# vmonardo/pnp-svrg

Measured on AMD Instinct MI355X. Metric: PnP-SVRG inner-iters/sec, 256x256 CSMRI+DnCNN, higher is better.
Workload: dtype f32; 1 GPU; pnp_svrg (true SVRG direction, T2=10, mb=1000) on 256x256 CSMRI, 20% Bernoulli mask, DnCNN-17 prox (reference DnCNN_noise15 weights); batch_per_gpu=120, problems_total=120, parallelism=replicas x1 (no data-path collective)

## Files before the change

### pnp_svrg_amd/csrc/dncnn.hip

```cpp
#include "direct.h"
#include "wino44.h"
#include "wino44b.h"
#include "reduce.h"
#include <vector>
#include <algorithm>
#include <cstdlib>
#include <type_traits>

namespace pnp {

constexpr int C = 64;

template <typename T>
__global__ __launch_bounds__(256) void k_first(const T* __restrict__ z, const T* __restrict__ mm,
                                               const float* __restrict__ w, const float* __restrict__ bfirst,
                                               float* __restrict__ out, int H, int W, double srange, double sshift,
                                               int clamp01, float slope) {
    __shared__ float ws[C * 9];
    __shared__ float bs[C];
    for (int i = threadIdx.x; i < C * 9; i += 256) ws[i] = w[i];
    if (threadIdx.x < C) bs[threadIdx.x] = bfirst[threadIdx.x];
    __syncthreads();
    const int b = blockIdx.y;
    const int p = blockIdx.x * 256 + threadIdx.x;
// ... 140 lines not shown
                                                      float blast) {
    __shared__ double red[4];
    const int tid = threadIdx.x, b = blockIdx.z;
    const int iy = tid >> 6, ix = tid & 3, bx = blockIdx.x * 16 + ((tid >> 2) & 15), by = blockIdx.y;
    const int y = 4 * by + iy, x = 4 * bx + ix;
    const int NBX = W / 4, NBY = H / 4;
    const float* pb = part + (size_t)b * NBY * NBX * 36;
    auto at = [&](int qy, int qx, int py, int px) { return pb[((size_t)qy * NBX + qx) * 36 + py * 6 + px]; };
    const int vy = iy == 0 ? -1 : iy == 3 ? 1 : 0, vx = ix == 0 ? -1 : ix == 3 ? 1 : 0;
    const bool hv = vy != 0 && by + vy >= 0 && by + vy < NBY, hh = vx != 0 && bx + vx >= 0 && bx + vx < NBX;
    const int py = iy + 1, px = ix + 1, pyn = py - 4 * vy, pxn = px - 4 * vx;
    float r = at(by, bx, py, px);
    if (hv) r += at(by + vy, bx, pyn, px);
    if (hh) r += at(by, bx + vx, py, pxn);
    if (hv && hh) r += at(by + vy, bx + vx, pyn, pxn);
    r += blast;
    const size_t p = (size_t)b * H * W + (size_t)y * W + x;
    if (r_out != nullptr) r_out[p] = r;
    double err = 0.0;
    if (zout != nullptr) {
        const T lo = mm ? mm[2 * b] : (T)0, hi = mm ? mm[2 * b + 1] : (T)1;
        T v = (zin[p] - lo) / (hi - lo);
        v = v * (T)srange + (T)sshift;
        v = v - (T)r;
        v = (v - (T)sshift) / (T)srange;
        v = v * (hi - lo) + lo;
        zout[p] = v;
        if (xrec != nullptr) {
            const double d = (double)xrec[p] - (double)v;
            err = d * d;
        }
    }
    if (sse_part != nullptr) {
        err = wave_sum(err);
        if ((tid & 63) == 0) red[tid >> 6] = err;
        __syncthreads();
        if (tid == 0)
            sse_part[((size_t)b * gridDim.y + blockIdx.y) * gridDim.x + blockIdx.x] = red[0] + red[1] + red[2] + red[3];
    }
}

__global__ void k_sum_parts(const double* __restrict__ part, int nparts, double* __restrict__ out) {
    double s = 0;
    for (int i = threadIdx.x; i < nparts; i += 64) s += part[(size_t)blockIdx.x * nparts + i];
    s = wave_sum(s);
    if (threadIdx.x == 0) out[blockIdx.x] = s;
}

}
using namespace pnp;

static const ConvMode kModes[] = {
    {0, direct_supports, direct_layer_bytes, direct_pack, direct_layer, direct_debug_clock, false},
    {1, direct_supports, wino23_layer_bytes, wino23_pack, wino23_layer, wino23_debug_clock, false},
    {5, wino44_supports, wino44_layer_bytes, wino44_pack, wino44_layer, wino44_debug_clock, true},
    {6, wino44b_supports, wino44b_layer_bytes, wino44b_pack, wino44b_layer, wino44b_debug_clock, false},
};
constexpr int NMODES = sizeof(kModes) / sizeof(kModes[0]);

static const ConvMode* find_mode(int mode) {
    for (const ConvMode& m : kModes)
        if (m.mode == mode) return &m;
    return nullptr;
}

static int resolve_conv_mode(int requested, int H, int W, bool strict, const ConvMode** out) {
    const ConvMode* m = find_mode(requested);
    PNP_CHECK_ARG(m || !strict,
                  "mode must be 0 (direct), 1 (Winograd F(2,3) along x), 5 (Winograd F(4x4,3x3)) or 6 (the same on 3 x bf16 splits)");
    if (!m) m = find_mode(5);
    PNP_CHECK_ARG(m->supports(H, W) || !strict, "Winograd F(4x4,3x3) needs H % 8 == 0 and W % 64 == 0");
    *out = m->supports(H, W) ? m : find_mode(1);
    return PNP_OK;
}

struct pnp_dncnn_plan {
    int n_mid, H, W, batch, num_cu;
    float *w_first, *w_last, *bias;
    void* wconv[NMODES];
    const ConvMode* conv;
    float* b_first;
    float b_last, slope;
    bool edge_fusion;
    float* part;
    float *act0, *act1, *zeros;
    double* mm;
    double* sse_part;
    bool profile;
    std::vector<hipEvent_t> ev;
    size_t ev_used;
    double prof_ms;
    long prof_launches;
};

static void plan_free(pnp_dncnn_plan* p) {
    for (void* q : p->wconv) (void)hipFree(q);
    for (void* q : {(void*)p->bias, (void*)p->w_first, (void*)p->w_last, (void*)p->act0, (void*)p->act1, (void*)p->zeros,
                    (void*)p->mm, (void*)p->sse_part, (void*)p->b_first, (void*)p->part})
        (void)hipFree(q);
    for (hipEvent_t e : p->ev) (void)hipEventDestroy(e);
    delete p;
}

static ConvLayerArgs conv_args(const pnp_dncnn_plan* p, int l, const float* in, float* out, hipStream_t s) {
    return {in, out, p->wconv[p->conv - kModes], l, p->bias + (size_t)l * C, p->zeros, p->H, p->W, p->batch, p->num_cu, p->slope, s};
}

extern "C" int pnp_dncnn_plan_create(pnp_dncnn_plan** out, int n_mid, const float* w_first, const float* w_mid,
                                     const float* b_mid, const float* w_last, int H, int W, int batch) {
    PNP_CHECK_ARG(out && w_first && w_mid && b_mid && w_last, "null argument");
    PNP_CHECK_ARG(n_mid >= 1 && batch >= 1, "n_mid and batch must be >= 1");
    PNP_CHECK_ARG(H % 8 == 0 && W % 32 == 0 && (H * W) % 256 == 0, "H must be a multiple of 8, W of 32");
    auto* p = new pnp_dncnn_plan{};
    p->n_mid = n_mid; p->H = H; p->W = W; p->batch = batch;
    hipDeviceProp_t prop;
    int dev = 0;
    PNP_CHECK_HIP(hipGetDevice(&dev));
    PNP_CHECK_HIP(hipGetDeviceProperties(&prop, dev));
    p->num_cu = prop.multiProcessorCount;
    const char* ev = getenv("PNP_DNCNN_WINOGRAD");
    (void)resolve_conv_mode(ev ? atoi(ev) : 5, H, W, false, &p->conv);
    const char* ef = getenv("PNP_DNCNN_EDGE_FUSION");
    p->edge_fusion = !(ef && atoi(ef) == 0);
    const size_t act_bytes = (size_t)batch * C * H * W * sizeof(float);
    hipError_t e = hipSuccess;
    auto alloc = [&](auto** dst, size_t bytes, const void* src = nullptr) {
        if (e == hipSuccess) e = hipMalloc(dst, bytes);
        if (e == hipSuccess && src) e = hipMemcpy(*dst, src, bytes, hipMemcpyHostToDevice);
    };
    for (int i = 0; i < NMODES; ++i) {
        if (!kModes[i].supports(H, W)) continue;
        std::vector<char> w(kModes[i].layer_bytes() * n_mid);
        kModes[i].pack(w_mid, n_mid, w.data());
        alloc(&p->wconv[i], w.size(), w.data());
    }
    alloc(&p->bias, (size_t)n_mid * C * sizeof(float), b_mid);
    alloc(&p->w_first, C * 9 * sizeof(float), w_first);
    alloc(&p->w_last, C * 9 * sizeof(float), w_last);
    alloc(&p->b_first, C * sizeof(float));
    if (e == hipSuccess) e = hipMemset(p->b_first, 0, C * sizeof(float));
    alloc(&p->act0, act_bytes);
    alloc(&p->act1, act_bytes);
    alloc(&p->zeros, 256);
    if (e == hipSuccess) e = hipMemset(p->zeros, 0, 256);
    alloc(&p->mm, (size_t)batch * 2 * sizeof(double));
    alloc(&p->sse_part, (size_t)batch * (H * W / 256) * sizeof(double));
    if (wino44_supports(H, W)) alloc(&p->part, wino44_part_floats(H, W, batch) * sizeof(float));
    if (e != hipSuccess) {
        set_error(std::string("pnp_dncnn_plan_create: ") + hipGetErrorString(e));
        plan_free(p);
        return PNP_ERR_HIP;
    }
    *out = p;
    return PNP_OK;
}

extern "C" int pnp_dncnn_plan_destroy(pnp_dncnn_plan* p) {
    if (p) plan_free(p);
    return PNP_OK;
}

namespace {
template <typename T>
int run_dncnn(pnp_dncnn_plan* p, const T* z_in, bool normalise, double sigma_net, T* z_out, float* r_out,
              const T* xrec, double* sse_out, hipStream_t s, bool mmo = false) {
    const int H = p->H, W = p->W, B = p->batch, HW = H * W;
    T* mm = normalise ? (T*)p->mm : nullptr;
    double srange = 1.0, sshift = 0.0;
    if (normalise) {
        k_minmax<T><<<B, 256, 0, s>>>(z_in, HW, mm);
        PNP_CHECK_LAUNCH();
        srange = 1.0 + sigma_net / 255.0 / 2.0;
        sshift = (1.0 - srange) / 2.0;
    }
    dim3 pg(HW / 256, B);
    k_first<T><<<pg, 256, 0, s>>>(z_in, mm, p->w_first, p->b_first, p->act0, H, W, srange, sshift, mmo ? 1 : 0, p->slope);
    PNP_CHECK_LAUNCH();
    float *src = p->act0, *dst = p->act1;
    const bool fuse_last = p->edge_fusion && p->conv->fuses_last && p->slope == 0.f && !mmo && std::is_same<T, float>::value &&
                           p->part != nullptr;
    const bool prof = p->profile && p->ev_used + 2 <= p->ev.size();
    if (prof) PNP_CHECK_HIP(hipEventRecord(p->ev[p->ev_used], s));
    for (int l = 0; l < p->n_mid; ++l) {
        ConvLayerArgs a = conv_args(p, l, src, dst, s);
        if (fuse_last && l == p->n_mid - 1) { a.wlast = p->w_last; a.part = p->part; }
        const int rc = p->conv->layer(a);
        if (rc != PNP_OK) return rc;
        std::swap(src, dst);
    }
    if (prof) { PNP_CHECK_HIP(hipEventRecord(p->ev[p->ev_used + 1], s)); p->ev_used += 2; }
    if (fuse_last) {
        const dim3 fg(W / 64, H / 4, B);
        k_last_patches<T><<<fg, 256, 0, s>>>(p->part, z_in, mm, z_out, r_out, xrec, sse_out ? p->sse_part : nullptr, H, W, srange,
                                             sshift, p->b_last);
        PNP_CHECK_LAUNCH();
        if (sse_out) {
            k_sum_parts<<<B, 64, 0, s>>>(p->sse_part, (int)(fg.x * fg.y), sse_out);
            PNP_CHECK_LAUNCH();
        }
        return PNP_OK;
    }
    dim3 lg((W + LT_C - 1) / LT_C, (H + LT_R - 1) / LT_R, B);
    k_last<T><<<lg, 256, 0, s>>>(src, p->w_last, z_in, mm, z_out, r_out, xrec, sse_out ? p->sse_part : nullptr, H, W,
                                 srange, sshift, mmo ? 1 : 0, p->b_last);
    PNP_CHECK_LAUNCH();
    if (sse_out) {
// ... 120 lines not shown
```

### pnp_svrg_amd/csrc/dncnn_conv.h

```cpp
#pragma once
#include "common.h"
#include <vector>

namespace pnp {

struct ConvLayerArgs {
    const float* in;
    float* out;
    const void* w;
    int layer;
    const float *bias, *zeros;
    int H, W, batch, num_cu;
    float slope;
    hipStream_t s;
    int force_rows = 0;
    const float* w44_override = nullptr;
    const float* wlast = nullptr;
    float* part = nullptr;
};

struct ConvMode {
    int mode;
    bool (*supports)(int H, int W);
    size_t (*layer_bytes)();
    void (*pack)(const float* w_mid, int n_mid, void* out);
    int (*layer)(const ConvLayerArgs& a);
    int (*debug_clock)(const ConvLayerArgs& a, int reps, std::vector<double>& cycles, std::vector<double>& ticks);
    bool fuses_last;
};

inline int check_plain_conv(const ConvLayerArgs& a) {
    PNP_CHECK_ARG(a.w44_override == nullptr, "w44_override needs the F(4x4,3x3) kernel (mode 5)");
    PNP_CHECK_ARG(a.part == nullptr, "the fused last layer needs the F(4x4,3x3) kernel (mode 5) and ReLU");
    return PNP_OK;
}

template <typename F>
int read_stamps(hipStream_t s, int nwg, int per_wg, F&& launch, std::vector<unsigned long long>& h, std::vector<double>& cycles,
                std::vector<double>& ticks) {
    unsigned long long* d = nullptr;
    PNP_CHECK_HIP(hipMalloc(&d, (size_t)nwg * per_wg * sizeof(*d)));
    h.resize((size_t)nwg * per_wg);
    const int rc = launch(d);
    hipError_t e = rc != PNP_OK ? hipSuccess : hipMemcpyAsync(h.data(), d, h.size() * sizeof(*d), hipMemcpyDeviceToHost, s);
    if (rc == PNP_OK && e == hipSuccess) e = hipStreamSynchronize(s);
    (void)hipFree(d);
    if (rc != PNP_OK) return rc;
    PNP_CHECK_HIP(e);
    for (int i = 0; i < nwg; ++i) { cycles.push_back((double)h[(size_t)per_wg * i]); ticks.push_back((double)h[(size_t)per_wg * i + 1]); }
    return PNP_OK;
}

}
```

### pnp_svrg_amd/csrc/dncnn_wino44.hip

```cpp
#include "common.h"
#include "wino44.h"
#include "wino44_common.h"
#include "tilewalk.h"
#include <vector>
#include <utility>
#include <cstdlib>

namespace pnp {
namespace w44 {

using namespace w44c;

template <int NG_> struct Geo : HaloGeo<NG_> {
    static constexpr int NG = NG_;
    static constexpr int VPL = 128 * NG;
    static constexpr int VBUF = 36 * VPL;
    static constexpr int LDS_FLOATS = 2 * HaloGeo<NG_>::DBUF + 2 * VBUF;
    static constexpr int NQ_AGPR = NG == 2 ? 64 : 36;
    static constexpr bool in_agpr(int g, int xi) { return g * 36 + xi < NQ_AGPR; }
};
constexpr int URING = 18;

#define PNP_MFMA_PRE ""
#define PNP_MFMA_POST ""
template <bool AG> __device__ __forceinline__ void mfma(f32x4& acc, float w, float v) {
    if (AG) asm volatile(PNP_MFMA_PRE "v_mfma_f32_16x16x4_f32 %0, %1, %2, %0" PNP_MFMA_POST : "+a"(acc) : "v"(w), "v"(v));
    else asm volatile(PNP_MFMA_PRE "v_mfma_f32_16x16x4_f32 %0, %1, %2, %0" PNP_MFMA_POST : "+v"(acc) : "v"(w), "v"(v));
}
template <bool AG> __device__ __forceinline__ void mfma_first(f32x4& acc, float w, float v) {
    if (AG) asm volatile("v_mfma_f32_16x16x4_f32 %0, %1, %2, 0" PNP_MFMA_POST : "=&a"(acc) : "v"(w), "v"(v));
    else asm volatile("v_mfma_f32_16x16x4_f32 %0, %1, %2, 0" PNP_MFMA_POST : "=&v"(acc) : "v"(w), "v"(v));
}

template <int NG_> struct Ctx : WeightCursor {
    static constexpr int NG = NG_;
    using G = Geo<NG_>;
    f32x4 acc[NG_][36];
    f32x4 ur[URING];
    Patch P;
    f32x2 b[2][NG_];
    const lds_f* dsrc[2];
    lds_f* vdst[2];
    const lds_f* vsrc0[2];
};
#define PNP_SLOT() __builtin_amdgcn_sched_barrier(0)

constexpr int col_pair(int sl) { return (sl - 6) / 2; }
constexpr bool is_col_slice(int sl) { return sl == 6 || sl == 8 || sl == 10; }
template <int SL, typename CT> __device__ __forceinline__ void slice_valu(CT& c) {
    Patch& P = c.P;
    if constexpr (SL < 6) {
        asm volatile("" :: "v"(P.a.x), "v"(P.e.y));
        const f32x2 p12 = {P.m.x, P.m.y}, p34 = {P.m.z, P.m.w};
        const f32x2 A = p34 - 4.f * p12;
        const f32x2 Bv = p34 - p12;
        P.t[SL][1] = pk_sum_diff(A);
        P.t[SL][2] = pk_hi_pm_2lo(Bv);
        float v0, v5;
        asm("v_fma_f32 %0, 4.0, %1, %2" : "=v"(v0) : "v"(P.a.y), "v"(__builtin_fmaf(-5.f, P.m.y, P.m.w)));
        asm("v_fma_f32 %0, 4.0, %1, %2" : "=v"(v5) : "v"(P.m.x), "v"(__builtin_fmaf(-5.f, P.m.z, P.e.x)));
        P.t[SL][0] = f32x2{v0, v5};
    } else if constexpr (is_col_slice(SL)) {
        constexpr int cp = col_pair(SL);
        bt6_pk(P.t[0][cp], P.t[1][cp], P.t[2][cp], P.t[3][cp], P.t[4][cp], P.t[5][cp], P.v);
    }
}
template <int DPAR, int SL, int Y, typename CT> __device__ __forceinline__ void v_write(CT& c) {
    constexpr int VPL = CT::G::VPL;
    constexpr int cp = col_pair(SL), xa = cp == 0 ? 0 : cp == 1 ? 1 : 3, xb = cp == 0 ? 5 : cp == 1 ? 2 : 4;
    c.vdst[DPAR][(Y * 6 + xa) * VPL] = c.P.v[Y].x;
    c.vdst[DPAR][(Y * 6 + xb) * VPL] = c.P.v[Y].y;
}
template <int DPAR, int SL, int N, typename CT> __device__ __forceinline__ void slice_lds(CT& c) {
    if constexpr (SL < 5) {
        if constexpr (N < 2) patch_load<DPAR, SL + 1, N>(c);
    } else if constexpr (is_col_slice(SL)) {
        v_write<DPAR, SL, 2 * N>(c);
        v_write<DPAR, SL, 2 * N + 1>(c);
    }
}
template <int VPAR, int XI, typename CT> __device__ __forceinline__ void b_load(CT& c) {
    if constexpr (CT::NG == 1) c.b[XI & 1][0] = *(const lds_f2*)(c.vsrc0[VPAR] + XI * CT::G::VPL);
    else {
        const f32x4 q = *(const lds_f4*)(c.vsrc0[VPAR] + XI * CT::G::VPL);
        c.b[XI & 1][0] = f32x2{q.x, q.y};
        c.b[XI & 1][CT::NG - 1] = f32x2{q.z, q.w};
    }
}
template <int K, int XI, int GR, typename CT> __device__ __forceinline__ void mfma_j0(CT& c, float u, f32x2 (&b)[CT::NG]) {
// ... 50 lines not shown
    else if constexpr (P == 7 || P == 9 || P == 11) slice_valu<P - 1>(c);
}
template <int K, int P, int VAR, typename CT, typename DMA> __device__ __forceinline__ void step2(CT& c, DMA&& dma) {
    static_assert(CT::NG == 2 && CT::G::PPW == 6, "one DMA piece in each of the steps 0..5");
    constexpr int X0 = 2 * P, X1 = 2 * P + 1, SQ = K * 18 + P;
    constexpr int VPAR = K & 1, DPAR = (K + 1) & 1;
    const f32x4 u = c.ur[SQ % URING];
    f32x2 b0[2] = {c.b[0][0], c.b[0][1]}, b1[2];
    mfma_j0<K, X0, 0>(c, u.x, b0);                   PNP_SLOT();
    if constexpr (VAR != 13 && VAR != 15) b_load<VPAR, X1>(c);
    PNP_SLOT();
    mfma_j0<K, X0, 1>(c, u.x, b0);                   PNP_SLOT();
    slot2<DPAR, P, 0, VAR>(c, dma);
    PNP_SLOT();
    mfma_j1<X0, 0>(c, u.y, b0);                      PNP_SLOT();
    if constexpr (VAR != 10 && VAR != 15) valu2<P>(c);
    if constexpr (P == 0 && K > 0 && VAR != 12 && VAR != 15 && SQ - 1 + URING < NCH * 18) c.ur[(SQ - 1) % URING] = c.uload_next();
    PNP_SLOT();
    mfma_j1<X0, 1>(c, u.y, b0);                      PNP_SLOT();
    slot2<DPAR, P, 1, VAR>(c, dma);
    PNP_SLOT();
    b1[0] = c.b[1][0]; b1[1] = c.b[1][1];
    mfma_j0<K, X1, 0>(c, u.z, b1);                   PNP_SLOT();
    if constexpr (X1 + 1 < 36 && VAR != 13 && VAR != 15) b_load<VPAR, X1 + 1>(c);
    PNP_SLOT();
    mfma_j0<K, X1, 1>(c, u.z, b1);                   PNP_SLOT();
    slot2<DPAR, P, 2, VAR>(c, dma);
    PNP_SLOT();
    mfma_j1<X1, 0>(c, u.w, b1);                      PNP_SLOT();
    slot2<DPAR, P, 3, VAR>(c, dma);
    PNP_SLOT();
    mfma_j1<X1, 1>(c, u.w, b1);                      PNP_SLOT();
    if constexpr (P < 17 && VAR != 12 && VAR != 15 && SQ + URING < NCH * 18) c.ur[SQ % URING] = c.uload_next();
    PNP_SLOT();
}
template <int K, int VAR, typename CT, typename DMA, int... P> __device__ __forceinline__ void chunk_steps(CT& c, DMA&& dma, std::integer_sequence<int, P...>) {
    if constexpr (CT::NG == 2) (step2<K, P, VAR>(c, dma), ...);
    else (step<K, P, VAR>(c, dma), ...);
}
template <int K> constexpr int reloads_of(int p0, int p1) {
    int n = 0;
    for (int p = p0; p <= p1; ++p) n += (K * 18 + p + URING < NCH * 18) ? 1 : 0;
    return n;
}
template <int K, bool STAMP, int VAR, typename CT, typename DMA> __device__ __forceinline__ void chunk(CT& c, DMA&& dma, unsigned long long& t_wait) {
    if constexpr (CT::NG == 1) {
        patch_load<(K + 1) & 1, 0, 0>(c);
        patch_load<(K + 1) & 1, 0, 1>(c);
    }
    b_load<K & 1, 0>(c);
    PNP_SLOT();
    chunk_steps<K, VAR>(c, dma, std::make_integer_sequence<int, 18>{});
    unsigned long long ta = 0;
    if (STAMP) ta = __builtin_amdgcn_s_memtime();
    constexpr int PPW = CT::G::PPW, younger = CT::NG == 2 ? reloads_of<K>(PPW - 1, 16) : reloads_of<K>(PPW, 17);
    asm volatile("s_waitcnt vmcnt(%0)" :: "n"(younger) : "memory");
    __syncthreads();
    if (STAMP) t_wait += __builtin_amdgcn_s_memtime() - ta;
}
template <bool STAMP, int VAR, typename CT, typename MK, int... K> __device__ __forceinline__ void all_chunks(CT& c, MK&& mk, unsigned long long& t_wait, std::integer_sequence<int, K...>) {
    (chunk<K, STAMP, VAR>(c, mk(std::integral_constant<int, K>{}), t_wait), ...);
}

template <int VPL> __device__ __forceinline__ void transform0(const float* dsrc, float* vdst) {
    float t[6][6];
#pragma unroll
    for (int r = 0; r < 6; ++r) {
        const float* row = dsrc + r * PC;
        bt6(row[3], row[4], row[5], row[6], row[7], row[8], t[r]);
    }
#pragma unroll
    for (int x = 0; x < 6; ++x) {
        float v[6];
        bt6(t[0][x], t[1][x], t[2][x], t[3][x], t[4][x], t[5][x], v);
#pragma unroll
        for (int y = 0; y < 6; ++y) vdst[(y * 6 + x) * VPL] = v[y];
    }
}

constexpr int FL_PATCH = 36;
constexpr int FL_BLK = 16 * FL_PATCH;
template <int NG, bool FL> constexpr int fl_lds_floats() { return FL ? C * 9 + NG * 4 * FL_BLK : 0; }

template <bool LEAKY, int NG = 2, bool STAMP = false, int VAR = 0, bool FL = false>
__global__ __launch_bounds__(256, 1) void k_mid_wino44(const float* __restrict__ in, float* __restrict__ out,
                                                       const float4* __restrict__ upack, const float* __restrict__ bias,
                                                       int H, int W, int ntiles, float slope,
                                                       unsigned long long* __restrict__ stamps = nullptr, int tile0 = 0,
                                                       const float* __restrict__ wlast = nullptr, float* __restrict__ part = nullptr) {
    using G = Geo<NG>;
    constexpr int PLANE = G::PLANE, DBUF = G::DBUF, PPW = G::PPW, VPL = G::VPL, VBUF = G::VBUF;
    static_assert(!(FL && LEAKY), "the fused last layer is built for the ReLU net");
    __shared__ __attribute__((aligned(16))) float lds[G::LDS_FLOATS + fl_lds_floats<NG, FL>()];
    const int tid = threadIdx.x, lane = tid & 63, wv = __builtin_amdgcn_readfirstlane(tid >> 6);
    const Regions<NG> region(H, W, tile0);

    float bv[4];
#pragma unroll
    for (int r = 0; r < 4; ++r) bv[r] = bias[16 * wv + 4 * (lane >> 4) + r];

    const int tc = lane & 15, j = (lane >> 4) & 1, g = NG == 2 ? lane >> 5 : 0;
    const int d_off = 4 * ((2 * wv + j) * (PLANE / 4) + g * PC + tc);
    const ptrdiff_t hw4 = (ptrdiff_t)4 * H * W, w4 = (ptrdiff_t)4 * W;
    const unsigned st_off = 4u * (unsigned)(4 * (lane >> 4) * H * W + 4 * tc);
    const int v_off = NG == 2 ? wv * 64 + tc * 4 + g * 2 + j : wv * 32 + tc * 2 + j;

    unsigned pdesc[PPW];
#pragma unroll
    for (int i = 0; i < PPW; ++i) pdesc[i] = piece_desc<NG>(wv, i, lane, H, W);
    const unsigned lds0 = (unsigned)(size_t)(__attribute__((address_space(3))) float*)lds;
    const size_t chunk_bytes = (size_t)KC * H * W * 4;
    auto tile_dma = [&](int t) {
        TileDma<NG> td;
        int b, ty0, tx0;
        region(t, b, ty0, tx0);
        td.base = (size_t)in + 4 * ((((size_t)b * C) * H + ty0 - 1) * (size_t)W + tx0 - 4);
        const unsigned bad = bad_mask<NG>(t, ntiles, ty0, tx0, H, W);
#pragma unroll
        for (int i = 0; i < PPW; ++i) td.voff[i] = piece_voff(pdesc[i], bad);
        return td;
    };

    float* const dbuf = lds;
    float* const vbuf = lds + 2 * DBUF;

    Ctx<NG> c;
    lds_f* const ldsp = (lds_f*)lds;
    c.dsrc[0] = ldsp + d_off;                     c.dsrc[1] = ldsp + DBUF + d_off;
    c.vdst[0] = ldsp + 2 * DBUF + v_off;          c.vdst[1] = ldsp + 2 * DBUF + VBUF + v_off;
    asm volatile("" : "+v"(c.vdst[0]), "+v"(c.vdst[1]));
    c.vsrc0[0] = ldsp + 2 * DBUF + 2 * NG * lane; c.vsrc0[1] = ldsp + 2 * DBUF + VBUF + 2 * NG * lane;
    const __attribute__((address_space(1))) char* const ubase = (const __attribute__((address_space(1))) char*)upack + (size_t)(wv * NCH * 18) * 1024;
    c.ucur = ubase;
    c.ulane = 16u * lane;

    const TileWalk tw_ = tile_walk(ntiles);
    int tile = tw_.first;
    const int limit = tw_.limit < ntiles ? tw_.limit : ntiles;
    float* const flw = lds + G::LDS_FLOATS;
    float* const flx = flw + C * 9;
    if constexpr (FL)
        for (int i = tid; i < C * 9; i += 256) flw[i] = wlast[i];
    {
        const TileDma<NG> td0 = tile_dma(tile < limit ? tile : ntiles);
#pragma unroll
        for (int i = 0; i < PPW; ++i) dma_piece(td0, chunk_rsrc(td0, 0, chunk_bytes), lds0, wv, 0, i);
#pragma unroll
        for (int i = 0; i < PPW; ++i) dma_piece(td0, chunk_rsrc(td0, 1, chunk_bytes), lds0, wv, 1, i);
#pragma unroll
        for (int i = 0; i < URING; ++i) c.ur[i] = c.uload_next();
        asm volatile("s_waitcnt vmcnt(0)" ::: "memory");
        __syncthreads();
        transform0<VPL>(dbuf + d_off, vbuf + v_off);
        __syncthreads();
    }

    unsigned long long t0 = 0, r0 = 0, t_wait = 0, t_epi = 0;
    if (STAMP) { t0 = __builtin_amdgcn_s_memtime(); r0 = __builtin_amdgcn_s_memrealtime(); }
    for (; tile < limit; tile += tw_.step) {
        asm volatile("" : "+v"(c.ulane));
        int b, ty0, tx0;
        region(tile, b, ty0, tx0);
        const int ntile = tile + tw_.step < limit ? tile + tw_.step : ntiles;

        const TileDma<NG> cur = tile_dma(tile), nxt = tile_dma(ntile);
        all_chunks<STAMP, VAR>(c, [&](auto kc) {
            constexpr int K = decltype(kc)::value;
            const TileDma<NG>& td = K + 2 < NCH ? cur : nxt;
            const i32x4 rs = chunk_rsrc(td, (K + 2) % NCH, chunk_bytes);
            return [&, rs](int piece) { dma_piece(td, rs, lds0, wv, K & 1, piece); };
        }, t_wait, std::make_integer_sequence<int, NCH>{});

        unsigned long long te = 0;
        if (STAMP) te = __builtin_amdgcn_s_memtime();
        asm volatile("; W44_EPILOGUE_BEGIN\n\ts_nop 15\n\ts_nop 7" ::: "memory");
#pragma unroll
        for (int g2 = 0; g2 < NG; ++g2)
#pragma unroll
            for (int xi = 0; xi < 36; xi += 4) {
                if (G::in_agpr(g2, xi)) asm volatile("" : "+a"(c.acc[g2][xi]), "+a"(c.acc[g2][xi + 1]), "+a"(c.acc[g2][xi + 2]), "+a"(c.acc[g2][xi + 3]));
                else asm volatile("" : "+v"(c.acc[g2][xi]), "+v"(c.acc[g2][xi + 1]), "+v"(c.acc[g2][xi + 2]), "+v"(c.acc[g2][xi + 3]));
            }
        unsigned so = st_off;
        asm volatile("" : "+v"(so));
        __attribute__((address_space(1))) char* const ob = (__attribute__((address_space(1))) char*)out + 4 * ((((size_t)b * C + 16 * wv) * H + ty0) * (size_t)W + tx0);
        float q[FL_PATCH];
#pragma unroll
        for (int blk = 0; blk < 2 * NG; ++blk) {
            {
                const int g2 = NG == 2 ? 1 - (blk >> 1) : 0, pi = blk & 1;
                float wr[2][9];
                if constexpr (FL) {
                    if (pi == 0)
#pragma unroll
                        for (int i = 0; i < FL_PATCH; ++i) q[i] = 0.f;
                    const float* wc = flw + (16 * wv + 4 * (lane >> 4) + 2 * pi) * 9;
#pragma unroll
                    for (int t = 0; t < 9; ++t) { wr[0][t] = wc[t]; wr[1][t] = wc[9 + t]; }
                }
                if (blk == 2 * NG - 1) {
                    c.ucur = ubase;
#pragma unroll
                    for (int i = 0; i < URING; ++i) c.ur[i] = c.uload_next();
                    __builtin_amdgcn_sched_barrier(0);
                }
                const f32x2 bias2 = {bv[2 * pi], bv[2 * pi + 1]};
                __attribute__((address_space(1))) char* oc = ob + (ptrdiff_t)(2 * pi) * hw4 + (ptrdiff_t)(4 * g2) * w4;
                asm volatile("" : "+s"(oc));
                f32x2 s[6][4];
#pragma unroll
                for (int x = 0; x < 6; ++x) {
                    f32x2 m[6];
#pragma unroll
                    for (int y = 0; y < 6; ++y) {
                        const f32x4 q = c.acc[g2][6 * y + x];
                        m[y] = pi ? f32x2{q.z, q.w} : f32x2{q.x, q.y};
                    }
                    if (x == 1) m[1] += bias2;
                    at6(m[0], m[1], m[2], m[3], m[4], m[5], s[x]);
                    if (x & 1) __builtin_amdgcn_sched_barrier(0);
                }
#pragma unroll
                for (int r = 0; r < 4; ++r) {
                    f32x2 y[4];
                    at6(s[0][r], s[1][r], s[2][r], s[3][r], s[4][r], s[5][r], y);
                    f32x4 v0, v1;
                    if (LEAKY) {
                        v0.x = fmaxf(y[0].x, slope * y[0].x); v0.y = fmaxf(y[1].x, slope * y[1].x);
                        v0.z = fmaxf(y[2].x, slope * y[2].x); v0.w = fmaxf(y[3].x, slope * y[3].x);
                        v1.x = fmaxf(y[0].y, slope * y[0].y); v1.y = fmaxf(y[1].y, slope * y[1].y);
                        v1.z = fmaxf(y[2].y, slope * y[2].y); v1.w = fmaxf(y[3].y, slope * y[3].y);
                    } else {
                        v0.x = fmaxf(y[0].x, 0.f); v0.y = fmaxf(y[1].x, 0.f); v0.z = fmaxf(y[2].x, 0.f); v0.w = fmaxf(y[3].x, 0.f);
                        v1.x = fmaxf(y[0].y, 0.f); v1.y = fmaxf(y[1].y, 0.f); v1.z = fmaxf(y[2].y, 0.f); v1.w = fmaxf(y[3].y, 0.f);
                    }
                    if constexpr (FL) {
                        const float a0[4] = {v0.x, v0.y, v0.z, v0.w}, a1[4] = {v1.x, v1.y, v1.z, v1.w};
#pragma unroll
                        for (int dy = 0; dy < 3; ++dy)
#pragma unroll
                            for (int dx = 0; dx < 3; ++dx)
#pragma unroll
                                for (int k = 0; k < 4; ++k) {
                                    float& d = q[(r + 2 - dy) * 6 + k + 2 - dx];
                                    d = __builtin_fmaf(wr[0][dy * 3 + dx], a0[k], d);
                                    d = __builtin_fmaf(wr[1][dy * 3 + dx], a1[k], d);
                                }
                    } else {
                        *(__attribute__((address_space(1))) f32x4*)(oc + so) = v0;
                        oc += hw4;
                        asm volatile("" : "+s"(oc));
                        *(__attribute__((address_space(1))) f32x4*)(oc + so) = v1;
                        oc += w4 - hw4;
                        asm volatile("" : "+s"(oc));
                    }
                    if (r & 1) __builtin_amdgcn_sched_barrier(0);
                }
                if constexpr (FL) {
                    if (pi == 1) {
                        const bool h32 = (lane & 32) != 0, h16 = (lane & 16) != 0;
                        float k1[18], k2[9];
#pragma unroll
                        for (int i = 0; i < 18; ++i) {
                            const float mine = h32 ? q[18 + i] : q[i], give = h32 ? q[i] : q[18 + i];
                            k1[i] = mine + __shfl_xor(give, 32);
                        }
#pragma unroll
                        for (int i = 0; i < 9; ++i) {
                            const float mine = h16 ? k1[9 + i] : k1[i], give = h16 ? k1[i] : k1[9 + i];
                            k2[i] = mine + __shfl_xor(give, 16);
                        }
                        float* const xd = flx + (g2 * 4 + wv) * FL_BLK + tc * FL_PATCH + 9 * (lane >> 4);
#pragma unroll
                        for (int i = 0; i < 9; ++i) xd[i] = k2[i];
                    }
                }
            }
        }
        if constexpr (FL) {
            __syncthreads();
            float* const pb = part + (((size_t)b * (H / 4) + ty0 / 4) * (size_t)(W / 4) + tx0 / 4) * FL_PATCH;
            for (int e = tid; e < NG * FL_BLK; e += 256) {
                const int g2 = e >= FL_BLK ? 1 : 0, rem = e - g2 * FL_BLK;
                const float* xs = flx + g2 * 4 * FL_BLK + rem;
                pb[(size_t)g2 * (W / 4) * FL_PATCH + rem] = ((xs[0] + xs[FL_BLK]) + xs[2 * FL_BLK]) + xs[3 * FL_BLK];
            }
        }
        asm volatile("; W44_EPILOGUE_END" ::: "memory");
        if (STAMP) t_epi += __builtin_amdgcn_s_memtime() - te;
    }
    if (STAMP && tid == 0) {
        stamps[4 * blockIdx.x] = __builtin_amdgcn_s_memtime() - t0;
        stamps[4 * blockIdx.x + 1] = __builtin_amdgcn_s_memrealtime() - r0;
        stamps[4 * blockIdx.x + 2] = t_wait;
        stamps[4 * blockIdx.x + 3] = t_epi;
    }
}

}

bool wino44_supports(int H, int W) { return H % 8 == 0 && W % w44::TC == 0; }

size_t wino44_layer_bytes() { return (size_t)4 * w44::NCH * 18 * 64 * 4 * sizeof(float); }

void wino44_pack(const float* w_mid, int n_mid, void* out_) {
    float* out = (float*)out_;
    for (int l = 0; l < n_mid; ++l)
        for (int wv = 0; wv < 4; ++wv)
            for (int k = 0; k < w44::NCH; ++k)
                for (int lane = 0; lane < 64; ++lane)
                    for (int j = 0; j < 2; ++j) {
                        const int cout = 16 * wv + (lane & 15), cin = w44::KC * k + 2 * (lane >> 4) + j;
                        const float* g = w_mid + (((size_t)l * w44::C + cout) * w44::C + cin) * 9;
                        float u[36];
                        w44c::filter_u(g, u);
                        for (int xi = 0; xi < 36; ++xi) {
                            const int p = xi >> 1, e = 2 * (xi & 1) + j;
                            out[((((size_t)(l * 4 + wv) * w44::NCH + k) * 18 + p) * 64 + lane) * 4 + e] = u[xi];
                        }
                    }
}

int wino44_layer(const ConvLayerArgs& a) {
    PNP_CHECK_ARG(a.part == nullptr || (a.slope == 0.f && a.wlast != nullptr), "the fused last layer needs ReLU and w_last");
    const float *in = a.in, *bias = a.bias, *wlast = a.wlast;
    float *out = a.out, *part = a.part;
    const int H = a.H, W = a.W, num_cu = a.num_cu, force = a.force_rows, batch = a.batch;
    const float slope = a.slope;
    const hipStream_t s = a.s;
    const int units = batch * (H / 8) * (W / w44::TC);
    int full = force == 1 ? 0 : force == 2 ? units : (units / num_cu) * num_cu;
    if (force == 0 && 2 * (units - full) > num_cu) full = units;
    const float4* up = (const float4*)(a.w44_override ? a.w44_override : (const float*)a.w + a.layer * wino44_layer_bytes() / sizeof(float));
    if (full > 0) {
        const int grid = full < num_cu ? full : num_cu;
        if (part) w44::k_mid_wino44<false, 2, false, 0, true><<<grid, 256, 0, s>>>(in, out, up, bias, H, W, full, 0.f, nullptr, 0, wlast, part);
        else if (slope != 0.f) w44::k_mid_wino44<true, 2><<<grid, 256, 0, s>>>(in, out, up, bias, H, W, full, slope, nullptr, 0);
        else w44::k_mid_wino44<false, 2><<<grid, 256, 0, s>>>(in, out, up, bias, H, W, full, 0.f, nullptr, 0);
        PNP_CHECK_LAUNCH();
    }
    if (full < units) {
        const int n1 = 2 * (units - full), grid = n1 < num_cu ? n1 : num_cu;
        if (part) w44::k_mid_wino44<false, 1, false, 0, true><<<grid, 256, 0, s>>>(in, out, up, bias, H, W, n1, 0.f, nullptr, full, wlast, part);
        else if (slope != 0.f) w44::k_mid_wino44<true, 1><<<grid, 256, 0, s>>>(in, out, up, bias, H, W, n1, slope, nullptr, full);
        else w44::k_mid_wino44<false, 1><<<grid, 256, 0, s>>>(in, out, up, bias, H, W, n1, 0.f, nullptr, full);
        PNP_CHECK_LAUNCH();
    }
    return PNP_OK;
}

int wino44_debug_clock(const ConvLayerArgs& a, int reps, std::vector<double>& cycles, std::vector<double>& ticks) {
    const int ntiles = a.batch * (a.H / 8) * (a.W / w44::TC);
    const int grid = ntiles < a.num_cu ? ntiles : a.num_cu;
    const float *in = a.in, *bias = a.bias;
    float* out = a.out;
    const int H = a.H, W = a.W;
    const hipStream_t s = a.s;
    const float* upack_layer = (const float*)a.w + a.layer * wino44_layer_bytes() / sizeof(float);
    std::vector<unsigned long long> h;
    const int rc = read_stamps(s, grid, 4, [&](unsigned long long* stamps_dev) {
        for (int i = 0; i < reps - 1; ++i)
            w44::k_mid_wino44<false, 2><<<grid, 256, 0, s>>>(in, out, (const float4*)upack_layer, bias, H, W, ntiles, 0.f);
        const int var = getenv("PNP_W44_VAR") ? atoi(getenv("PNP_W44_VAR")) : 0;
        if (var == 0) w44::k_mid_wino44<false, 2, true><<<grid, 256, 0, s>>>(in, out, (const float4*)upack_layer, bias, H, W, ntiles, 0.f, stamps_dev);
#ifdef PNP_W44_ABLATIONS
#define PNP_W44_ABL(V) else if (var == V) w44::k_mid_wino44<false, 2, true, V><<<grid, 256, 0, s>>>(in, out, (const float4*)upack_layer, bias, H, W, ntiles, 0.f, stamps_dev);
        PNP_W44_ABL(10) PNP_W44_ABL(11) PNP_W44_ABL(12) PNP_W44_ABL(13) PNP_W44_ABL(14) PNP_W44_ABL(15)
#undef PNP_W44_ABL
#endif
        else PNP_CHECK_ARG(false, "PNP_W44_VAR: this library was built without -DPNP_W44_ABLATIONS");
        PNP_CHECK_LAUNCH();
        return PNP_OK;
    }, h, cycles, ticks);
    if (rc != PNP_OK) return rc;
    if (getenv("PNP_DEBUG_STAMPS")) w44c::print_stamp_summary("k_mid_wino44", h, grid);
    return PNP_OK;
}

}
```

### pnp_svrg_amd/csrc/tilewalk.h

```cpp
#pragma once

namespace pnp {

struct TileWalk { int first, step, limit; };

__device__ __forceinline__ TileWalk tile_walk(int ntiles) {
    const int G = (int)gridDim.x, bid = (int)blockIdx.x;
    if ((G & 7) == 0 && ntiles % G == 0) {
        const int per_xcd = ntiles >> 3, xcd = bid & 7, slot = bid >> 3;
        return {xcd * per_xcd + slot, G >> 3, (xcd + 1) * per_xcd};
    }
    return {bid, G, ntiles};
}

}
```

### pnp_svrg_amd/csrc/wino44_common.h

```cpp
#pragma once
#include "common.h"
#include <vector>
#include <cstdio>

namespace pnp {
namespace w44c {

using f32x4 = __attribute__((ext_vector_type(4))) float;
using f32x2 = __attribute__((ext_vector_type(2))) float;
typedef int i32x4 __attribute__((ext_vector_type(4)));
typedef __attribute__((address_space(3))) float lds_f;
typedef __attribute__((address_space(3))) f32x2 lds_f2;
typedef __attribute__((address_space(3))) f32x4 lds_f4;

constexpr int C = 64;
constexpr int TC = 64;
constexpr int PC = 72;
constexpr int KC = 8;
constexpr int NCH = C / KC;
constexpr unsigned DUMMY = 1u << 27;
template <int NG> struct HaloGeo {
    static constexpr int TR = 4 * NG, PR = TR + 2;
    static constexpr int PLANE = NG == 2 ? 768 : 512;
    static constexpr int DBUF = KC * PLANE;
// ... 29 lines not shown
}
__device__ __forceinline__ void bt6_pk(f32x2 q0, f32x2 q1, f32x2 q2, f32x2 q3, f32x2 q4, f32x2 q5, f32x2 (&v)[6]) {
    const f32x2 t1 = q4 - 4.f * q2, t2 = q3 - 4.f * q1;
    const f32x2 t3 = q4 - q2, sd = q3 - q1;
    v[0] = 4.f * q0 + (q4 - 5.f * q2);
    v[1] = t1 + t2;
    v[2] = t1 - t2;
    v[3] = 2.f * sd + t3;
    v[4] = t3 - 2.f * sd;
    v[5] = 4.f * q1 + (q5 - 5.f * q3);
}

struct Patch {
    f32x2 a; f32x4 m; f32x2 e;
    f32x2 t[6][3];
    f32x2 v[6];
};
template <int DPAR, int R, int HALF, typename CT> __device__ __forceinline__ void patch_load(CT& c) {
    const lds_f* row = c.dsrc[DPAR] + R * PC;
    if (HALF == 0) { c.P.a = *(const lds_f2*)(row + 2); c.P.e = *(const lds_f2*)(row + 8); }
    else c.P.m = *(const lds_f4*)(row + 4);
}
struct WeightCursor {
    const __attribute__((address_space(1))) char* ucur;
    unsigned ulane;
    __device__ __forceinline__ f32x4 uload_next() {
        const f32x4 u = *(const __attribute__((address_space(1))) f32x4*)(ucur + ulane);
        ucur += 1024;
        asm volatile("" : "+s"(ucur));
        return u;
    }
};

__device__ __forceinline__ void dma_piece_asm(unsigned voff, i32x4 rsrc, unsigned lds_byte_addr) {
    asm volatile("s_mov_b32 m0, %2\n\ts_nop 0\n\tbuffer_load_dwordx4 %0, %1, 0 offen lds" :: "v"(voff), "s"(rsrc), "s"(lds_byte_addr) : "memory");
}

template <int NG> struct Regions {
    int tile0, tiles_x, units_per_img;
    __device__ __forceinline__ Regions(int H, int W, int tile0_) : tile0(tile0_), tiles_x(W / TC), units_per_img(tiles_x * (H / 8)) {}
    __device__ __forceinline__ void operator()(int u, int& b, int& ty0, int& tx0) const {
        const int t = tile0 + (NG == 2 ? u : u >> 1);
        b = t / units_per_img;
        const int t2 = t - b * units_per_img;
        ty0 = (t2 / tiles_x) * 8 + (NG == 2 ? 0 : 4 * (u & 1));
        tx0 = (t2 % tiles_x) * TC;
    }
};
template <int NG> __device__ __forceinline__ unsigned piece_desc(int wv, int i, int lane, int H, int W) {
    using G = HaloGeo<NG>;
    const int q = (wv + 4 * i) * 64 + lane;
    const int c = q / (G::PLANE / 4), r = q - c * (G::PLANE / 4);
    const int ry = r / 18, cx4 = 4 * (r - ry * 18);
    const unsigned edge = (ry == 0 ? 1u : 0u) | (ry == G::PR - 1 ? 2u : 0u) | (cx4 == 0 ? 4u : 0u) | (cx4 == TC + 4 ? 8u : 0u);
    return r < G::PR * 18 ? ((unsigned)((c * H + ry) * W + cx4) | (edge << 28)) : DUMMY;
}
template <int NG> struct TileDma { size_t base; unsigned voff[HaloGeo<NG>::PPW]; };
template <int NG> __device__ __forceinline__ unsigned bad_mask(int t, int ntiles, int ty0, int tx0, int H, int W) {
    return t < ntiles ? ((((ty0 == 0 ? 1u : 0u) | (ty0 + HaloGeo<NG>::TR == H ? 2u : 0u) | (tx0 == 0 ? 4u : 0u) | (tx0 + TC == W ? 8u : 0u)) << 28) | DUMMY)
                      : 0xFFFFFFFFu;
}
__device__ __forceinline__ unsigned piece_voff(unsigned pdesc, unsigned bad) { return (pdesc & bad) == 0u ? 4u * (pdesc & 0x07FFFFFFu) : 0x80000000u; }
template <int NG> __device__ __forceinline__ i32x4 chunk_rsrc(const TileDma<NG>& td, int k, size_t chunk_bytes) {
    const size_t base = td.base + (size_t)k * chunk_bytes;
    i32x4 rs;
    rs.x = (int)(unsigned)base; rs.y = (int)(unsigned)(base >> 32) & 0xFFFF; rs.z = (int)0x80000000u; rs.w = 0x00020000;
    return rs;
}
template <int NG> __device__ __forceinline__ void dma_piece(const TileDma<NG>& td, i32x4 rs, unsigned lds0, int wv, int buf, int i) {
    dma_piece_asm(td.voff[i], rs, lds0 + 4u * (unsigned)(buf * HaloGeo<NG>::DBUF + (wv + 4 * i) * 256));
}

inline void filter_u(const float* g, float (&u)[36]) {
    static const double G[6][3] = {{1.0 / 4, 0, 0}, {-1.0 / 6, -1.0 / 6, -1.0 / 6}, {-1.0 / 6, 1.0 / 6, -1.0 / 6},
                                   {1.0 / 24, 1.0 / 12, 1.0 / 6}, {1.0 / 24, -1.0 / 12, 1.0 / 6}, {0, 0, 1}};
    for (int xy = 0; xy < 6; ++xy)
        for (int xx = 0; xx < 6; ++xx) {
            double s = 0;
            for (int dy = 0; dy < 3; ++dy)
                for (int dx = 0; dx < 3; ++dx) s += G[xy][dy] * G[xx][dx] * (double)g[dy * 3 + dx];
            u[6 * xy + xx] = (float)s;
        }
}
inline void print_stamp_summary(const char* kernel, const std::vector<unsigned long long>& h, int grid) {
    double wsum = 0, esum = 0, rsum = 0;
    for (int i = 0; i < grid; ++i) { wsum += (double)(h[4 * i + 2] & 0xFFFFFFFFull); rsum += (double)(h[4 * i + 2] >> 32); esum += h[4 * i + 3]; }
    fprintf(stderr, "[%s stamps] mean cycles per WG: chunk-end wait + barrier %.0f  epilogue %.0f  (mode 6: steps 0..5 of the chunks %.0f)\n",
            kernel, wsum / grid, esum / grid, rsum / grid);
}

}
}
```

Baseline: 5341 inner-iters/s.

## Reverse the tile walk on alternate Winograd layers and overlap the prologue loads

Even-numbered mid layers now walk their tiles in reverse within each XCD slice, so each layer starts on the tiles the previous layer wrote last and those are more likely still in L2/MALL. The prologue is also reordered: weight-ring loads are issued between the two halo DMA chunks, last-layer weights are staged in registers and written to LDS, and the first transform waits only on the first chunk rather than on all outstanding loads. Extra launch-edge timestamps and a diagnostic printer are added for debugging. The change adds index-mirroring arithmetic and relies on the reversal matching the previous layer's write order.

```diff
diff --git a/pnp_svrg_amd/csrc/dncnn.hip b/pnp_svrg_amd/csrc/dncnn.hip
--- a/pnp_svrg_amd/csrc/dncnn.hip
+++ b/pnp_svrg_amd/csrc/dncnn.hip
@@ -246,6 +246,7 @@
     float* b_first;
     float b_last, slope;
     bool edge_fusion;
+    bool reverse_walk;
     float* part;
     float *act0, *act1, *zeros;
     double* mm;
@@ -267,7 +268,9 @@
 }
 
 static ConvLayerArgs conv_args(const pnp_dncnn_plan* p, int l, const float* in, float* out, hipStream_t s) {
-    return {in, out, p->wconv[p->conv - kModes], l, p->bias + (size_t)l * C, p->zeros, p->H, p->W, p->batch, p->num_cu, p->slope, s};
+    ConvLayerArgs a{in, out, p->wconv[p->conv - kModes], l, p->bias + (size_t)l * C, p->zeros, p->H, p->W, p->batch, p->num_cu, p->slope, s};
+    a.reverse_walk = p->reverse_walk;
+    return a;
 }
 
 extern "C" int pnp_dncnn_plan_create(pnp_dncnn_plan** out, int n_mid, const float* w_first, const float* w_mid,
@@ -286,6 +289,8 @@
     (void)resolve_conv_mode(ev ? atoi(ev) : 5, H, W, false, &p->conv);
     const char* ef = getenv("PNP_DNCNN_EDGE_FUSION");
     p->edge_fusion = !(ef && atoi(ef) == 0);
+    const char* rw = getenv("PNP_W44_REVERSE_WALK");
+    p->reverse_walk = !(rw && atoi(rw) == 0);
     const size_t act_bytes = (size_t)batch * C * H * W * sizeof(float);
     hipError_t e = hipSuccess;
     auto alloc = [&](auto** dst, size_t bytes, const void* src = nullptr) {
diff --git a/pnp_svrg_amd/csrc/dncnn_conv.h b/pnp_svrg_amd/csrc/dncnn_conv.h
--- a/pnp_svrg_amd/csrc/dncnn_conv.h
+++ b/pnp_svrg_amd/csrc/dncnn_conv.h
@@ -17,6 +17,7 @@
     const float* w44_override = nullptr;
     const float* wlast = nullptr;
     float* part = nullptr;
+    bool reverse_walk = false;
 };
 
 struct ConvMode {
diff --git a/pnp_svrg_amd/csrc/dncnn_wino44.hip b/pnp_svrg_amd/csrc/dncnn_wino44.hip
--- a/pnp_svrg_amd/csrc/dncnn_wino44.hip
+++ b/pnp_svrg_amd/csrc/dncnn_wino44.hip
@@ -5,6 +5,7 @@
 #include <vector>
 #include <utility>
 #include <cstdlib>
+#include <algorithm>
 
 namespace pnp {
 namespace w44 {
@@ -221,15 +222,19 @@
 constexpr int FL_BLK = 16 * FL_PATCH;
 template <int NG, bool FL> constexpr int fl_lds_floats() { return FL ? C * 9 + NG * 4 * FL_BLK : 0; }
 
+constexpr int STAMP_WORDS = 7;
 template <bool LEAKY, int NG = 2, bool STAMP = false, int VAR = 0, bool FL = false>
 __global__ __launch_bounds__(256, 1) void k_mid_wino44(const float* __restrict__ in, float* __restrict__ out,
                                                        const float4* __restrict__ upack, const float* __restrict__ bias,
                                                        int H, int W, int ntiles, float slope,
                                                        unsigned long long* __restrict__ stamps = nullptr, int tile0 = 0,
-                                                       const float* __restrict__ wlast = nullptr, float* __restrict__ part = nullptr) {
+                                                       const float* __restrict__ wlast = nullptr, float* __restrict__ part = nullptr,
+                                                       int reverse = 0) {
     using G = Geo<NG>;
     constexpr int PLANE = G::PLANE, DBUF = G::DBUF, PPW = G::PPW, VPL = G::VPL, VBUF = G::VBUF;
     static_assert(!(FL && LEAKY), "the fused last layer is built for the ReLU net");
+    unsigned long long t_in = 0, r_in = 0;
+    if (STAMP) { t_in = __builtin_amdgcn_s_memtime(); r_in = __builtin_amdgcn_s_memrealtime(); }
     __shared__ __attribute__((aligned(16))) float lds[G::LDS_FLOATS + fl_lds_floats<NG, FL>()];
     const int tid = threadIdx.x, lane = tid & 63, wv = __builtin_amdgcn_readfirstlane(tid >> 6);
     const Regions<NG> region(H, W, tile0);
@@ -273,24 +278,38 @@
     c.ucur = ubase;
     c.ulane = 16u * lane;
 
-    const TileWalk tw_ = tile_walk(ntiles);
+    const DirectedWalk tw_ = tile_walk(ntiles, reverse != 0);
     int tile = tw_.first;
     const int limit = tw_.limit < ntiles ? tw_.limit : ntiles;
     float* const flw = lds + G::LDS_FLOATS;
     float* const flx = flw + C * 9;
-    if constexpr (FL)
-        for (int i = tid; i < C * 9; i += 256) flw[i] = wlast[i];
+    float wl[(C * 9 + 255) / 256];
+    if constexpr (FL) {
+#pragma unroll
+        for (int i = 0; i < (C * 9 + 255) / 256; ++i) wl[i] = tid + 256 * i < C * 9 ? wlast[tid + 256 * i] : 0.f;
+        __builtin_amdgcn_sched_barrier(0);
+    }
     {
-        const TileDma<NG> td0 = tile_dma(tile < limit ? tile : ntiles);
+        const TileDma<NG> td0 = tile_dma(tile < limit ? tw_.at(tile) : ntiles);
 #pragma unroll
         for (int i = 0; i < PPW; ++i) dma_piece(td0, chunk_rsrc(td0, 0, chunk_bytes), lds0, wv, 0, i);
+        __builtin_amdgcn_sched_barrier(0);
+#pragma unroll
+        for (int i = 0; i < URING; ++i) c.ur[i] = c.uload_next();
+        __builtin_amdgcn_sched_barrier(0);
 #pragma unroll
         for (int i = 0; i < PPW; ++i) dma_piece(td0, chunk_rsrc(td0, 1, chunk_bytes), lds0, wv, 1, i);
-#pragma unroll
-        for (int i = 0; i < URING; ++i) c.ur[i] = c.uload_next();
-        asm volatile("s_waitcnt vmcnt(0)" ::: "memory");
+        __builtin_amdgcn_sched_barrier(0);
+        if constexpr (FL) {
+#pragma unroll
+            for (int i = 0; i < (C * 9 + 255) / 256; ++i)
+                if (tid + 256 * i < C * 9) flw[tid + 256 * i] = wl[i];
+            __builtin_amdgcn_sched_barrier(0);
+        }
+        asm volatile("s_waitcnt vmcnt(%0)" :: "n"(URING + PPW) : "memory");
         __syncthreads();
         transform0<VPL>(dbuf + d_off, vbuf + v_off);
+        asm volatile("s_waitcnt vmcnt(0)" ::: "memory");
         __syncthreads();
     }
 
@@ -299,10 +318,11 @@
     for (; tile < limit; tile += tw_.step) {
         asm volatile("" : "+v"(c.ulane));
         int b, ty0, tx0;
-        region(tile, b, ty0, tx0);
-        const int ntile = tile + tw_.step < limit ? tile + tw_.step : ntiles;
-
-        const TileDma<NG> cur = tile_dma(tile), nxt = tile_dma(ntile);
+        const int rtile = tw_.at(tile);
+        region(rtile, b, ty0, tx0);
+        const int ntile = tile + tw_.step < limit ? tw_.at(tile + tw_.step) : ntiles;
+
+        const TileDma<NG> cur = tile_dma(rtile), nxt = tile_dma(ntile);
         all_chunks<STAMP, VAR>(c, [&](auto kc) {
             constexpr int K = decltype(kc)::value;
             const TileDma<NG>& td = K + 2 < NCH ? cur : nxt;
@@ -429,10 +449,15 @@
         if (STAMP) t_epi += __builtin_amdgcn_s_memtime() - te;
     }
     if (STAMP && tid == 0) {
-        stamps[4 * blockIdx.x] = __builtin_amdgcn_s_memtime() - t0;
-        stamps[4 * blockIdx.x + 1] = __builtin_amdgcn_s_memrealtime() - r0;
-        stamps[4 * blockIdx.x + 2] = t_wait;
-        stamps[4 * blockIdx.x + 3] = t_epi;
+        const unsigned long long r1 = __builtin_amdgcn_s_memrealtime();
+        unsigned long long* const st = stamps + (size_t)STAMP_WORDS * blockIdx.x;
+        st[0] = __builtin_amdgcn_s_memtime() - t0;
+        st[1] = r1 - r0;
+        st[2] = t_wait;
+        st[3] = t_epi;
+        st[4] = t0 - t_in;
+        st[5] = r1;
+        st[6] = r_in;
     }
 }
 
@@ -467,25 +492,58 @@
     const int H = a.H, W = a.W, num_cu = a.num_cu, force = a.force_rows, batch = a.batch;
     const float slope = a.slope;
     const hipStream_t s = a.s;
+    const int rev = a.reverse_walk && (a.layer & 1) == 0 ? 1 : 0;
     const int units = batch * (H / 8) * (W / w44::TC);
     int full = force == 1 ? 0 : force == 2 ? units : (units / num_cu) * num_cu;
     if (force == 0 && 2 * (units - full) > num_cu) full = units;
     const float4* up = (const float4*)(a.w44_override ? a.w44_override : (const float*)a.w + a.layer * wino44_layer_bytes() / sizeof(float));
     if (full > 0) {
         const int grid = full < num_cu ? full : num_cu;
-        if (part) w44::k_mid_wino44<false, 2, false, 0, true><<<grid, 256, 0, s>>>(in, out, up, bias, H, W, full, 0.f, nullptr, 0, wlast, part);
-        else if (slope != 0.f) w44::k_mid_wino44<true, 2><<<grid, 256, 0, s>>>(in, out, up, bias, H, W, full, slope, nullptr, 0);
-        else w44::k_mid_wino44<false, 2><<<grid, 256, 0, s>>>(in, out, up, bias, H, W, full, 0.f, nullptr, 0);
+        if (part) w44::k_mid_wino44<false, 2, false, 0, true><<<grid, 256, 0, s>>>(in, out, up, bias, H, W, full, 0.f, nullptr, 0, wlast, part, rev);
+        else if (slope != 0.f) w44::k_mid_wino44<true, 2><<<grid, 256, 0, s>>>(in, out, up, bias, H, W, full, slope, nullptr, 0, nullptr, nullptr, rev);
+        else w44::k_mid_wino44<false, 2><<<grid, 256, 0, s>>>(in, out, up, bias, H, W, full, 0.f, nullptr, 0, nullptr, nullptr, rev);
         PNP_CHECK_LAUNCH();
     }
     if (full < units) {
-        const int n1 = 2 * (units - full), grid = n1 < num_cu ? n1 : num_cu;
-        if (part) w44::k_mid_wino44<false, 1, false, 0, true><<<grid, 256, 0, s>>>(in, out, up, bias, H, W, n1, 0.f, nullptr, full, wlast, part);
-        else if (slope != 0.f) w44::k_mid_wino44<true, 1><<<grid, 256, 0, s>>>(in, out, up, bias, H, W, n1, slope, nullptr, full);
-        else w44::k_mid_wino44<false, 1><<<grid, 256, 0, s>>>(in, out, up, bias, H, W, n1, 0.f, nullptr, full);
+        const int n1 = 2 * (units - full), grid = n1 < num_cu ? n1 : num_cu, rev1 = full > 0 ? 0 : rev;
+        if (part) w44::k_mid_wino44<false, 1, false, 0, true><<<grid, 256, 0, s>>>(in, out, up, bias, H, W, n1, 0.f, nullptr, full, wlast, part, rev1);
+        else if (slope != 0.f) w44::k_mid_wino44<true, 1><<<grid, 256, 0, s>>>(in, out, up, bias, H, W, n1, slope, nullptr, full, nullptr, nullptr, rev1);
+        else w44::k_mid_wino44<false, 1><<<grid, 256, 0, s>>>(in, out, up, bias, H, W, n1, 0.f, nullptr, full, nullptr, nullptr, rev1);
         PNP_CHECK_LAUNCH();
     }
     return PNP_OK;
+}
+
+static void print_launch_edges(const std::vector<unsigned long long>& h, int grid) {
+    const int W = w44::STAMP_WORDS;
+    double pro = 0, pro_max = 0, loop = 0, loop_max = 0, cyc = 0, exit_mean = 0, xcd_loop[8] = {}, xcd_exit[8] = {};
+    int xcd_n[8] = {};
+    unsigned long long first_in = ~0ull, last_in = 0, first_out = ~0ull, last_out = 0;
+    for (int i = 0; i < grid; ++i) {
+        const unsigned long long* w = h.data() + (size_t)W * i;
+        first_in = std::min(first_in, w[6]); last_in = std::max(last_in, w[6]);
+        first_out = std::min(first_out, w[5]); last_out = std::max(last_out, w[5]);
+    }
+    for (int i = 0; i < grid; ++i) {
+        const unsigned long long* w = h.data() + (size_t)W * i;
+        pro += (double)w[4]; pro_max = std::max(pro_max, (double)w[4]);
+        loop += (double)w[1]; loop_max = std::max(loop_max, (double)w[1]);
+        cyc += (double)w[0];
+        exit_mean += (double)(w[5] - first_in);
+        xcd_loop[i & 7] += (double)w[1]; xcd_exit[i & 7] += (double)(w[5] - first_in); ++xcd_n[i & 7];
+    }
+    pro /= grid; loop /= grid; cyc /= grid; exit_mean /= grid;
+    const double ghz = cyc / loop * 0.1, us = 0.01;
+    fprintf(stderr, "[k_mid_wino44 launch edges] %d workgroups, shader clock %.3f GHz\n", grid, ghz);
+    fprintf(stderr, "  prologue (kernel entry -> tile loop): mean %.0f cycles = %.2f us, max %.0f cycles = %.2f us\n", pro, pro / ghz * 1e-3,
+            pro_max, pro_max / ghz * 1e-3);
+    fprintf(stderr, "  tile loop: mean %.2f us, max %.2f us; per XCD mean", loop * us, loop_max * us);
+    for (int x = 0; x < 8; ++x) fprintf(stderr, " %.2f", xcd_n[x] ? xcd_loop[x] / xcd_n[x] * us : 0.0);
+    fprintf(stderr, " us\n  loop exit after the first kernel entry: mean %.2f us, last %.2f us, exit skew (last - mean) %.2f us; per XCD mean",
+            exit_mean * us, (double)(last_out - first_in) * us, ((double)(last_out - first_in) - exit_mean) * us);
+    for (int x = 0; x < 8; ++x) fprintf(stderr, " %.2f", xcd_n[x] ? xcd_exit[x] / xcd_n[x] * us : 0.0);
+    fprintf(stderr, " us\n  kernel entries spread over %.2f us, loop exits over %.2f us; first entry -> last exit %.2f us\n",
+            (double)(last_in - first_in) * us, (double)(last_out - first_out) * us, (double)(last_out - first_in) * us);
 }
 
 int wino44_debug_clock(const ConvLayerArgs& a, int reps, std::vector<double>& cycles, std::vector<double>& ticks) {
@@ -497,7 +555,7 @@
     const hipStream_t s = a.s;
     const float* upack_layer = (const float*)a.w + a.layer * wino44_layer_bytes() / sizeof(float);
     std::vector<unsigned long long> h;
-    const int rc = read_stamps(s, grid, 4, [&](unsigned long long* stamps_dev) {
+    const int rc = read_stamps(s, grid, w44::STAMP_WORDS, [&](unsigned long long* stamps_dev) {
         for (int i = 0; i < reps - 1; ++i)
             w44::k_mid_wino44<false, 2><<<grid, 256, 0, s>>>(in, out, (const float4*)upack_layer, bias, H, W, ntiles, 0.f);
         const int var = getenv("PNP_W44_VAR") ? atoi(getenv("PNP_W44_VAR")) : 0;
@@ -512,7 +570,10 @@
         return PNP_OK;
     }, h, cycles, ticks);
     if (rc != PNP_OK) return rc;
-    if (getenv("PNP_DEBUG_STAMPS")) w44c::print_stamp_summary("k_mid_wino44", h, grid);
+    if (getenv("PNP_DEBUG_STAMPS")) {
+        w44c::print_stamp_summary("k_mid_wino44", h, grid, w44::STAMP_WORDS);
+        print_launch_edges(h, grid);
+    }
     return PNP_OK;
 }
 
diff --git a/pnp_svrg_amd/csrc/tilewalk.h b/pnp_svrg_amd/csrc/tilewalk.h
--- a/pnp_svrg_amd/csrc/tilewalk.h
+++ b/pnp_svrg_amd/csrc/tilewalk.h
@@ -13,4 +13,19 @@
     return {bid, G, ntiles};
 }
 
+struct DirectedWalk {
+    int first, step, limit;
+    int mirror;
+    __device__ __forceinline__ int at(int t) const { return mirror >= 0 ? mirror - t : t; }
+};
+
+__device__ __forceinline__ DirectedWalk tile_walk(int ntiles, bool reverse) {
+    const int G = (int)gridDim.x, bid = (int)blockIdx.x;
+    if ((G & 7) == 0 && ntiles % G == 0) {
+        const int per_xcd = ntiles >> 3, xcd = bid & 7, slot = bid >> 3;
+        return {xcd * per_xcd + slot, G >> 3, (xcd + 1) * per_xcd, reverse ? (2 * xcd + 1) * per_xcd - 1 : -1};
+    }
+    return {bid, G, ntiles, reverse ? ntiles - 1 : -1};
 }
+
+}
diff --git a/pnp_svrg_amd/csrc/wino44_common.h b/pnp_svrg_amd/csrc/wino44_common.h
--- a/pnp_svrg_amd/csrc/wino44_common.h
+++ b/pnp_svrg_amd/csrc/wino44_common.h
@@ -135,9 +135,12 @@
             u[6 * xy + xx] = (float)s;
         }
 }
-inline void print_stamp_summary(const char* kernel, const std::vector<unsigned long long>& h, int grid) {
+inline void print_stamp_summary(const char* kernel, const std::vector<unsigned long long>& h, int grid, int per_wg = 4) {
     double wsum = 0, esum = 0, rsum = 0;
-    for (int i = 0; i < grid; ++i) { wsum += (double)(h[4 * i + 2] & 0xFFFFFFFFull); rsum += (double)(h[4 * i + 2] >> 32); esum += h[4 * i + 3]; }
+    for (int i = 0; i < grid; ++i) {
+        const unsigned long long* w = h.data() + (size_t)per_wg * i;
+        wsum += (double)(w[2] & 0xFFFFFFFFull); rsum += (double)(w[2] >> 32); esum += w[3];
+    }
     fprintf(stderr, "[%s stamps] mean cycles per WG: chunk-end wait + barrier %.0f  epilogue %.0f  (mode 6: steps 0..5 of the chunks %.0f)\n",
             kernel, wsum / grid, esum / grid, rsum / grid);
 }
```

Result: no change. 5340 inner-iters/s (-0.0%).
